# takah29/2d-fluid-simulator

Hardware: AMD Instinct MI355X
Metric: simulation steps/sec + Poisson-sweep HBM GB/s (% roofline), res 4096², 1/2/4/8 GPU (higher is better)
Workload: dtype f32; 1 GPU; bc=5 res=4096 (8192x4096 cells) scheme=cip vc=5.0 RB-SOR(1.3, 2 iters) Re=1e+06 dt=0.05/res; BASELINE.json configs[2]; cells=33554432, fluid_cells=22424499, parallelism=y-slab x1

## Files before the change

### 2d-fluid-simulator_amd/csrc/fs_core.hip

```cpp
#include <algorithm>
#include <cstdio>
#include <cstdlib>
#include <cstring>
#include <cxxabi.h>
#include <mutex>
#include <numeric>
#include <type_traits>
#include <unordered_map>

#include "fs_launch.h"
#include "fs_tracer.h"

namespace fs {

static thread_local std::string g_err;
void set_error(const std::string &msg) { g_err = msg; }
int no_variant(const char *name)
{
    set_error(std::string(name) + ": no kernel variant for these arguments");
    return FS_ERR_UNSUPPORTED;
}
int hip_fail(hipError_t e, const char *what, const char *file, int line)
{
    char buf[512];
// ... 88 lines not shown
        c->prof_ms[r.name_id] += ms;
        c->prof_pool.push_back(r.start);
        c->prof_pool.push_back(r.stop);
    }
    c->prof_recs.clear();
    return FS_OK;
}

const fs_ctx::TileList *tile_list(fs_ctx *c, TileSpec spec)
{
    if (c->act.quad.empty() || !tile_spec_ok(spec, c->rows)) return nullptr;
    const fs_ctx::TileKey key = spec.key();
    auto it = c->tile_lists.find(key);
    if (it != c->tile_lists.end()) return it->second.d ? &it->second : nullptr;
    if (c->capturing || c->tape_rec || c->tile_lists.size() >= 512) { ++c->tile_list_misses; return nullptr; }
    const TileWords h = build_tile_list(spec, c->act.of(spec.lanes).data(), c->X, c->rows);
    fs_ctx::TileList tl;
    if (h.needed) {
        if (hipMalloc(&tl.d, h.words.size() * sizeof(uint32_t)) == hipSuccess &&
            hipMemcpyAsync(tl.d, h.words.data(), h.words.size() * sizeof(uint32_t), hipMemcpyHostToDevice, c->stream) == hipSuccess &&
            hipStreamSynchronize(c->stream) == hipSuccess)
            { tl.per_xcd = h.per_xcd; tl.count = h.count; }
        else { if (tl.d) hipFree(tl.d); tl.d = nullptr; }
    }
    auto &slot = c->tile_lists[key] = tl;
    return slot.d ? &slot : nullptr;
}

static void tile_lists_free(fs_ctx *c)
{
    for (auto &kv : c->tile_lists) if (kv.second.d) hipFree(kv.second.d);
    c->tile_lists.clear();
}

int check_rows(const fs_ctx *c, int jb, int je)
{
    if (!(0 <= jb && jb <= je && je <= c->rows)) {
// ... 474 lines not shown
    FS_HIP(hipSetDevice(ctx->device));
    FS_HIP(hipMemsetAsync(ctx->d_mask, 1, (size_t)ctx->rows * ctx->Pm, ctx->stream));
    int rc = upload_global(ctx, ctx->d_mask, 1, 1, mask_xy, ctx->Pm);
    if (rc) return rc;
    rc = build_bc_ops(ctx, mask_xy);
    if (rc) return rc;
    if (!ctx->d_bcmap) FS_HIP(hipMalloc(&ctx->d_bcmap, (size_t)ctx->rows * ctx->Pm));
    if (!ctx->d_lazyflags) FS_HIP(hipMalloc(&ctx->d_lazyflags, (size_t)std::max(ctx->nwx, 1) * ctx->rows));
    FS_HIP(hipMemsetAsync(ctx->d_bcmap, 0, (size_t)ctx->rows * ctx->Pm, ctx->stream));
    FS_HIP(hipMemsetAsync(ctx->d_lazyflags, 63, (size_t)std::max(ctx->nwx, 1) * ctx->rows, ctx->stream));
    rc = upload_global(ctx, ctx->d_bcmap, 1, 1, ctx->h_bcmap.data(), ctx->Pm);
    for (auto &gexec : ctx->graphs) if (gexec) { hipGraphExecDestroy(gexec); gexec = nullptr; }
    for (auto &tp : ctx->tapes) if (tp) { delete tp; tp = nullptr; }
    tile_lists_free(ctx);
    ctx->act.clear();
    if (ctx->X % 2 == 0 && ctx->tile_list_mask && ctx->rows <= TILE_MAX_ROWS)
        ctx->act = activity_maps(mask_xy, ctx->h_bcmap.data(), ctx->X, ctx->Y, ctx->rows, ctx->y0 - ctx->halo);
    std::vector<uint8_t>().swap(ctx->h_bcmap);
    if (rc) return rc;
    if (ctx->X % 4 == 0) {
        klaunch(k_lazy_flags, dim3((ctx->nwx * ctx->rows + 3) / 4), dim3(256), ctx->stream, ctx->grid(), ctx->nwx, ctx->d_bcmap, ctx->d_lazyflags);
        FS_HIP(hipGetLastError());
        const size_t cap = (size_t)ctx->nwx * ctx->rows;
        if (!ctx->d_pairlist) FS_HIP(hipMalloc(&ctx->d_pairlist, (2 * cap + 2) * sizeof(uint32_t)));
        unsigned *d_count = (unsigned *)(ctx->d_pairlist + 2 * cap);
        FS_HIP(hipMemsetAsync(d_count, 0, 2 * sizeof(unsigned), ctx->stream));
        klaunch(k_pair_list, dim3((ctx->nwx * ctx->rows + 3) / 4), dim3(256), ctx->stream, ctx->grid(), ctx->nwx, (uint8_t *)ctx->d_lazyflags,
                           ctx->d_pairlist, ctx->d_pairlist + cap, d_count);
        FS_HIP(hipGetLastError());
        unsigned n[2] = {0, 0};
        FS_HIP(hipMemcpyAsync(n, d_count, 2 * sizeof(unsigned), hipMemcpyDeviceToHost, ctx->stream));
        FS_HIP(hipStreamSynchronize(ctx->stream));
// ... 1189 lines not shown
    FS_REQUIRE(ctx->span_ev[0], "fs_span_end without fs_span_begin");
    FS_HIP(hipEventRecord(ctx->span_ev[1], ctx->stream));
    FS_HIP(hipEventSynchronize(ctx->span_ev[1]));
    float f = 0.f;
    FS_HIP(hipEventElapsedTime(&f, ctx->span_ev[0], ctx->span_ev[1]));
    *ms = f;
    return FS_OK;
}

int fs_prof_reset(fs_ctx *ctx)
{
    FS_REQUIRE(ctx, "ctx is null");
    int rc = prof_drain(ctx); if (rc) return rc;
    std::fill(ctx->prof_launches.begin(), ctx->prof_launches.end(), 0);
    std::fill(ctx->prof_ms.begin(), ctx->prof_ms.end(), 0.0);
    return FS_OK;
}

int fs_prof_count(fs_ctx *ctx, int *n)
{
    FS_REQUIRE(ctx && n, "null argument");
    int rc = prof_drain(ctx); if (rc) return rc;
    *n = (int)ctx->prof_names.size();
    return FS_OK;
}

int fs_prof_get(fs_ctx *ctx, int idx, char *name, int name_cap, int *launches, double *total_ms)
{
    FS_REQUIRE(ctx, "ctx is null");
    FS_REQUIRE(idx >= 0 && idx < (int)ctx->prof_names.size(), "bad profile index");
// ... 38 lines not shown
```

### 2d-fluid-simulator_amd/csrc/fs_host.h

```cpp
#pragma once
#include <hip/hip_runtime.h>
#include <stdint.h>

#include <array>
#include <cmath>
#include <functional>
#include <map>
#include <set>
#include <string>
#include <vector>

#include "../../include/fs_hip.h"
#include "fs_device.h"
#include "fs_kernels.h"
#include "fs_march.h"
#include "fs_rbpair.h"
#include "fs_jquad.h"
#include "fs_k34n.h"
#include "fs_history.h"

namespace fs {

void set_error(const std::string &msg);
int hip_fail(hipError_t e, const char *what, const char *file, int line);
// ... 98 lines not shown
    std::set<fs_tracer *> tracers;
    std::vector<std::function<void()>> deferred_release;
    void release_deferred()
    {
        for (auto &release : deferred_release) release();
        deferred_release.clear();
    }
    bool use_march = true;
    bool use_pairs = true;
    int fuse_k2 = 2;
    bool limit_gate = true;
    int stack_mask = 0;

    int tile_list_mask = 1 | 2 | 4 | 8 | 32;
    fs::ActivityMaps act;
    struct TileList { uint32_t *d = nullptr; int per_xcd = 0; int count = 0; };
    using TileKey = decltype(fs::TileSpec().key());
    std::map<TileKey, TileList> tile_lists;

    fs::Grid grid() const
    {
        fs::Grid g;
        g.tiles = nullptr;
        g.X = X; g.P = P; g.Pm = Pm; g.rows = rows;
        int jlo = halo - y0, jhi = halo - y0 + (Y - 1);
        g.jlo = jlo < 0 ? 0 : jlo;
        g.jhi = jhi > rows - 1 ? rows - 1 : jhi;
        g.ybase = y0 - halo;
        g.mask = d_mask;
        return g;
    }
// ... 136 lines not shown
```

### 2d-fluid-simulator_amd/csrc/fs_k234.h

```cpp
#pragma once
#include <type_traits>

#include "fs_k34n.h"

namespace fs {

#if defined(__HIP_DEVICE_COMPILE__)
#define FS_PIN_LANE_OFFSET(i) asm volatile("" : "+v"(i))
#else
#define FS_PIN_LANE_OFFSET(i) (void)(i)
#endif

template <int RT> struct K234State {
    v2f Nn[RT + 4], Fc[RT + 4], GX[RT + 2], GY[RT + 2];
};

template <int c, int RT, int DM>
__device__ __forceinline__ void k234_nonadv(const Grid &g, const Konst<float> &k, const LaneMapN<2> &lm, int i0, int j0,
                                            const float *fc, const float *pc, K234State<RT> &st)
{
    using T = float;
    constexpr int N = 2;
    v2f F[RT + 6];
    v2f P[RT + 6];
// ... 129 lines not shown
    const int lane = threadIdx.x & 63;
    cip_k34_pk_core<2, c, RT, DM, false, false>(g, k, lm, i0, j0, je, MaskPacked{nwbits >> 2, flbits}, st.Nn, st.Fc, st.GX, st.GY, AdvLds<RT>{xch + (1 - c) * (RT + 2), lane}, out, gxo, gyo, hot, gxc, gyc);
}

#ifndef FS_K234_BND_WAVES
#define FS_K234_BND_WAVES 4
#endif
template <int RT, int DM>
__global__ __launch_bounds__(128, FS_K234_BND_WAVES) void k_cip_step_bnd(Grid g, Konst<float> k, int nbx, int nby, int jb, int je,
                                                      float *out, float *gxo, float *gyo, float *fn, const float *fc, const float *pc,
                                                      const float *gxc, const float *gyc, unsigned *hot, unsigned *hot_fn)
{
    constexpr int N = 2, HL = 2, OW = 64 - 2 * HL;
    __shared__ v2f xch[2 * (RT + 2)][64];
    int wx, ty, cg;
    if (!band_coords<1>(g, nbx, nby, wx, ty, cg)) return;
    if (!(wx * OW < g.X / N && jb + ty * RT < je)) return;
    const int c = __builtin_amdgcn_readfirstlane((int)(threadIdx.x >> 6));
    const LaneMapN<N> lm = lane_map_n<N, HL>(g, wx);
    const int i0 = lm.i0, j0 = jb + ty * RT;
    K234State<RT> st;
    unsigned nwbits, flbits;
    if (c == 0) k234_bnd_phase1<0, RT, DM>(g, k, lm, i0, j0, je, fn, fc, pc, gxc, gyc, hot_fn, st, nwbits, flbits, xch);
    else        k234_bnd_phase1<1, RT, DM>(g, k, lm, i0, j0, je, fn, fc, pc, gxc, gyc, hot_fn, st, nwbits, flbits, xch);
    __syncthreads();
    if (c == 0) k234_bnd_phase2<0, RT, DM>(g, k, lm, i0, j0, je, out, gxo, gyo, gxc, gyc, hot, st, nwbits, flbits, xch);
    else        k234_bnd_phase2<1, RT, DM>(g, k, lm, i0, j0, je, out, gxo, gyo, gxc, gyc, hot, st, nwbits, flbits, xch);
}

template <int RT, int DM>
__global__ __launch_bounds__(128, 4) void k_cip_step_all(Grid g, Konst<float> k, int nbx, int nby, int jb, int je,
                                                         float *out, float *gxo, float *gyo, float *fn, const float *fc, const float *pc,
                                                         const float *gxc, const float *gyc, unsigned *hot, unsigned *hot_fn)
{
    constexpr int N = 2, HL = 2, OW = 64 - 2 * HL;
    __shared__ v2f xch[2 * (RT + 2)][64];
    int wx, ty, cg;
    unsigned cls = 0u;
    if (!band_coords<1>(g, nbx, nby, wx, ty, cg, 0, &cls)) return;
    if (!(wx * OW < g.X / N && jb + ty * RT < je)) return;
    const int c = __builtin_amdgcn_readfirstlane((int)(threadIdx.x >> 6));
    const LaneMapN<N> lm_in = lane_map_n<N, HL>(g, wx);
    const int i0 = lm_in.i0, j0 = jb + ty * RT;
    K234State<RT> st;
    if (cls & 1u) {
        const LaneMapN<N> lm{lm_in.i0, lm_in.owner, false, false};
        if (c == 0) k234_phase1<0, RT, DM>(g, k, lm, i0, j0, fc, pc, gxc, gyc, st, xch);
        else        k234_phase1<1, RT, DM>(g, k, lm, i0, j0, fc, pc, gxc, gyc, st, xch);
        __syncthreads();
        if (c == 0) k234_phase2<0, RT, DM>(g, k, lm, i0, j0, je, out, gxo, gyo, hot, st, xch);
        else        k234_phase2<1, RT, DM>(g, k, lm, i0, j0, je, out, gxo, gyo, hot, st, xch);
    } else {
        unsigned nwbits, flbits;
        if (c == 0) k234_bnd_phase1<0, RT, DM>(g, k, lm_in, i0, j0, je, fn, fc, pc, gxc, gyc, hot_fn, st, nwbits, flbits, xch);
        else        k234_bnd_phase1<1, RT, DM>(g, k, lm_in, i0, j0, je, fn, fc, pc, gxc, gyc, hot_fn, st, nwbits, flbits, xch);
        __syncthreads();
        if (c == 0) k234_bnd_phase2<0, RT, DM>(g, k, lm_in, i0, j0, je, out, gxo, gyo, gxc, gyc, hot, st, nwbits, flbits, xch);
// ... 116 lines not shown
```

### 2d-fluid-simulator_amd/csrc/fs_launch.h

```cpp
#pragma once
#include <algorithm>
#include <cstdio>
#include <cstdlib>
#include <cstring>
#include <type_traits>

#include "fs_host.h"
#include "fs_pick.h"

namespace fs {

hipEvent_t prof_event(fs_ctx *c);


template <typename F>
inline bool launched(const F &f)
{
    if constexpr (std::is_void<decltype(f())>::value) { f(); return true; }
    else return f();
}
int no_variant(const char *name);

template <typename F>
inline int launch(fs_ctx *c, const char *name, F &&f)
// ... 78 lines not shown
    klaunch(kern, og.grid, dim3(og.threads), stream, og.g, k, og.nbx, og.nby, args...);
}
template <typename... P, typename... A>
inline void klaunch(void (*kern)(Grid, int, int, P...), const OvGrid &og, hipStream_t stream, A... args)
{
    klaunch(kern, og.grid, dim3(og.threads), stream, og.g, og.nbx, og.nby, args...);
}
enum { XCD_RBSOR = 1, XCD_VORT = 2, XCD_ADVECT = 4, XCD_NONADV = 8, XCD_GRAD = 16, XCD_JACOBI = 32 };

struct TileLaunch {
    int family, lanes;
    int rt = 1, zgroups = 1, wgw = 4;
    bool compact = true;
    int cls = TILES_ALL, reach = 0, parent_rt = 0;
    bool slab_classes = false;

    TileLaunch rows(int n) const { TileLaunch l = *this; l.rt = n; return l; }
    TileLaunch channel_groups(int n) const { TileLaunch l = *this; l.zgroups = n; return l; }
    TileLaunch waves(int n) const { TileLaunch l = *this; l.wgw = n; return l; }
    TileLaunch dense_if(bool dense) const { TileLaunch l = *this; l.compact = !dense; return l; }
    TileLaunch hints_within(int reach_) const { TileLaunch l = *this; l.cls = TILES_ALL; l.reach = reach_; return l; }
    TileLaunch plain_within(int reach_) const { TileLaunch l = *this; l.cls = TILES_PLAIN; l.reach = reach_; return l; }
    TileLaunch boundary_within(int reach_) const { TileLaunch l = *this; l.cls = TILES_BOUNDARY; l.reach = reach_; return l; }
    TileLaunch mixed_within(int reach_) const { TileLaunch l = *this; l.cls = TILES_MIXED; l.reach = reach_; return l; }
    TileLaunch parent_rows(int n) const { TileLaunch l = *this; l.parent_rt = n; return l; }
    TileLaunch classes_on_slabs(bool on) const { TileLaunch l = *this; l.slab_classes = on; return l; }
};
static inline TileLaunch tiles(int family, int lanes) { return TileLaunch{family, lanes}; }

static inline TileLaunch one_wave_where_hinted(const fs_ctx *c, TileLaunch l)
{
    if (c->dtype == 0 && (l.family & (XCD_RBSOR | XCD_JACOBI)) && l.wgw == 4 && l.cls == TILES_ALL && l.reach > 0 && l.compact) l.wgw = 1;
    return l;
}
static inline TileSpec list_spec(const fs_ctx *c, const TileLaunch &l, int jb, int je)
{
    TileSpec s;
    s.lanes = l.lanes; s.rt = l.rt; s.wgw = l.wgw; s.cls = l.cls; s.reach = l.reach; s.parent_rt = l.parent_rt; s.jb = jb; s.je = je;
    const int waves = geo_waves(c->X, l.lanes), tile_rows = (je - jb + l.rt - 1) / l.rt;
    s.stacked = (c->stack_mask & l.family) != 0 && l.wgw > 1;
    s.nbx = s.stacked ? waves : (waves + l.wgw - 1) / l.wgw;
    s.nby = s.stacked ? (tile_rows + l.wgw - 1) / l.wgw : tile_rows;
    constexpr int xg = 8;
    s.group = s.stacked ? std::max(1, xg / l.wgw) : xg;
    return s;
}
const fs_ctx::TileList *tile_list(fs_ctx *c, TileSpec spec);

static inline OvGrid ov_grid(fs_ctx *c, int jb, int je, const TileLaunch &asked)
{
    const TileLaunch l = one_wave_where_hinted(c, asked);
    const TileSpec s = list_spec(c, l, jb, je);
    OvGrid o;
// ... 38 lines not shown
```

### 2d-fluid-simulator_amd/csrc/fs_march.h

```cpp
#pragma once
#include "fs_device.h"
#include "fs_kernels.h"
#include "fs_tiles.h"

namespace fs {

template <typename T> struct Quad;
template <> struct Quad<float> { using type = float4; };
template <> struct Quad<double> { using type = double4; };

__device__ __forceinline__ float lane_prev(float x)
{ return __int_as_float(__builtin_amdgcn_update_dpp(0, __float_as_int(x), 0x138, 0xf, 0xf, true)); }
__device__ __forceinline__ float lane_next(float x)
{ return __int_as_float(__builtin_amdgcn_update_dpp(0, __float_as_int(x), 0x130, 0xf, 0xf, true)); }
__device__ __forceinline__ double lane_prev(double x)
{
    const int lo = __builtin_amdgcn_update_dpp(0, __double2loint(x), 0x138, 0xf, 0xf, true), hi = __builtin_amdgcn_update_dpp(0, __double2hiint(x), 0x138, 0xf, 0xf, true);
    return __hiloint2double(hi, lo);
}
__device__ __forceinline__ double lane_next(double x)
{
    const int lo = __builtin_amdgcn_update_dpp(0, __double2loint(x), 0x130, 0xf, 0xf, true), hi = __builtin_amdgcn_update_dpp(0, __double2hiint(x), 0x130, 0xf, 0xf, true);
    return __hiloint2double(hi, lo);
}
// ... 69 lines not shown
__device__ __forceinline__ void source_from(const Konst<T> &k, T vxE, T vxW, T vyE, T vyW, T vxN, T vxS, T vyN, T vyS, T &s2, T &s3)
{
    T sxx = vxE - vxW, sxy = vyE - vyW, syx = vxN - vxS, syy = vyN - vyS;
    s2 = ((sxx * sxx + syy * syy) + (syx * sxy)) / (T)8.0;
    s3 = cdiv<DM>(k.dx * (sxx + syy), k.eight_dt, k.r_eight_dt);
}

struct LaneMap {
    int i0;
    bool owner;
    bool at_lo;
    bool at_hi;
};
constexpr int FS_CG_INNER = 1 << 22;
template <int ZG = 1>
__device__ __forceinline__ bool band_coords(const Grid &g, int nbx, int nby_packed, int &bx, int &by, int &cg, int zoff = 0, unsigned *cls = nullptr)
{
    if (cls) *cls = 0u;
    if (g.tiles) {
        const int t = (int)blockIdx.x >> 3, xcd = (int)blockIdx.x & 7;
        const int k = ZG == 1 ? t : t / ZG;
        cg = ZG == 1 ? 0 : t - k * ZG;
        const uint32_t e = g.tiles[k * 8 + xcd];
        bx = tile_entry_bx(e);
        by = tile_entry_by(e);
        if (cls) *cls = tile_entry_hints(e);
        return e != TILE_PAD;
    }
    const int nby = nby_packed & 0x3fffff, FS_XCD_GROUP = (nby_packed >> 24) + 1;
    const int xcd = blockIdx.x & 7;
    int ly;
    if (ZG > 1 && (nby_packed & FS_CG_INNER)) {
        const int t = (int)blockIdx.x >> 3;
        bx = t / ZG;
        cg = t - bx * ZG;
        ly = (int)blockIdx.y;
    } else {
        bx = blockIdx.x >> 3;
        ly = ZG == 1 ? (int)blockIdx.y : (int)blockIdx.y / ZG;
        cg = ZG == 1 ? 0 : (int)blockIdx.y - ly * ZG;
    }
// ... 726 lines not shown
```

### 2d-fluid-simulator_amd/csrc/fs_pressure.hip

```cpp
#include "fs_launch.h"

using namespace fs;

template <bool SW, bool HV, typename T>
static bool launch_pair(fs_ctx *ctx, const OvGrid &og, int rt, int row_begin, int row_end, fs_field *pn, const fs_field *pc, const fs_field *src)
{
    const uint32_t *list = ctx->d_pairlist + (HV ? (size_t)ctx->nwx * ctx->rows : 0);
    const int nlist = ctx->n_pairlist[HV ? 1 : 0];
    const int per_slice = (int)(og.grid.x * og.grid.y), blocks = nlist, zoff = (blocks + per_slice - 1) / per_slice;
    const dim3 grid(og.grid.x, og.grid.y, og.grid.z + zoff);
    return pick<2, 3>(rt, [&](auto RT) {
        klaunch(k_jacobi_pair<RT, SW, HV, T>, grid, dim3(256), ctx->stream, og.g, og.nbx, og.nby, row_begin, row_end, (const uint8_t *)ctx->d_bcmap,
                (const uint8_t *)ctx->d_lazyflags, list, nlist, zoff, (T *)pn->d, (const T *)pc->d, (const T *)src->d);
    });
}

template <bool SRC, typename T>
static int launch_jacobi(fs_ctx *ctx, const char *name, const Konst<T> &k, int jb, int je, T *pn, const T *pc, const T *vs)
{
    if constexpr (!SRC && std::is_same<T, float>::value) {
        if (ctx->use_pairs) {
            const OvGrid og = ov_grid(ctx, jb, je, tiles(XCD_JACOBI, LANES_PAIR_WIDE).rows(4).hints_within(1));
            const int dm = dm_const(ctx, k);
            return launch(ctx, name, [=] { return with_dm_const<T>(dm, [&](auto DM) { klaunch(k_jacobi_ov2<4, DM>, og, ctx->stream, k, jb, je, pn, pc, vs); }); });
// ... 200 lines not shown
            const OvGrid ogb = ov_grid(ctx, row_begin, row_end, tiles(XCD_RBSOR, LANES_PAIR).rows(2).waves(1).boundary_within(4).parent_rows(4));
            if (ogp.g.tiles && ogb.g.tiles) {
                int rc = launch(ctx, "rbsor_pair", [=] { return run(ogp, Int<4>{}, Int<3>{}, Bool<false>{}); });
                if (rc) return rc;
                return launch(ctx, "rbsor_pair_bnd", [=] { return run(ogb, Int<2>{}, Int<2>{}, Bool<false>{}); });
            }
        }
        const OvGrid og = ov_grid(ctx, row_begin, row_end, tiles(XCD_RBSOR, LANES_PAIR).rows(2).dense_if(full).hints_within(4));
        return launch(ctx, "rbsor_pair", [=] { return pick_bool(full != 0, [&](auto FULL) { return run(og, Int<2>{}, Int<2>{}, FULL); }); });
    }
    using T = float;
    auto k = make_konst<T>(ctx, dt, dx, 1.0, 0.0, omega);
    const int dm = dm_const(ctx, k);
    const int rt = full || !small_tiles(ctx) ? 4 : 2;
    if (!full && split_launch(ctx, (size_t)ctx->X * ctx->Y, (size_t)1 << 20)) {
        const OvGrid og = ov_grid(ctx, row_begin, row_end, tiles(XCD_RBSOR, LANES_PAIR).rows(8).waves(1).mixed_within(4).parent_rows(16).classes_on_slabs(ctx->halo != 0));
        if (og.g.tiles) {
            return launch(ctx, "rbsor_pair", [=] {
                return pick<0, 1>(par0, [&](auto PAR) { return with_dm_const<T>(dm, [&](auto DM) {
                    klaunch(k_rbsor_pair_all<2, PAR, DM, T>, og.with_threads(128), ctx->stream, k, row_begin, row_end, (const uint8_t *)ctx->d_bcmap, (T *)pc_out->d, (T *)pn_out->d,
                            (const T *)pc->d, (const T *)pn->d, (const T *)vc->d);
                }); });
            });
        }
    }
    const OvGrid og = ov_grid(ctx, row_begin, row_end, tiles(XCD_RBSOR, LANES_PAIR).rows(rt).dense_if(full).hints_within(4));
    auto run = [=](auto RT, auto DM, auto FULL) {
        constexpr int tile = decltype(RT)::value, mode = decltype(DM)::value;
        constexpr bool carry = decltype(FULL)::value;
        return pick<0, 1>(par0, [&](auto PAR) {
            klaunch(k_rbsor_pair<2, tile, PAR, mode, 2, carry, T>, og, ctx->stream, k, row_begin, row_end, (const uint8_t *)ctx->d_bcmap, (T *)pc_out->d, (T *)pn_out->d,
// ... 76 lines not shown
```

### 2d-fluid-simulator_amd/csrc/fs_rbpair.h

```cpp
#pragma once
#include "fs_march.h"

namespace fs {

#ifndef FS_RBP_MIRROR
#define FS_RBP_MIRROR 1
#endif

template <typename T, int N> struct LV { T a[N]; };
template <typename T, int N> struct LVec;
template <> struct LVec<float, 4> { using type = float4; };
template <> struct LVec<float, 2> { using type = float2; };
template <> struct LVec<double, 2> { using type = double2; };
template <int N> struct LMaskWord;
template <> struct LMaskWord<4> { using type = uint32_t; };
template <> struct LMaskWord<2> { using type = uint16_t; };

template <typename T, int N>
__device__ __forceinline__ LV<T, N> lv_load(const T *row, int i0)
{
    const typename LVec<T, N>::type q = load_row_quad<typename LVec<T, N>::type, T>(row, i0);
    LV<T, N> r;
    if constexpr (N == 4) { r.a[0] = q.x; r.a[1] = q.y; r.a[2] = q.z; r.a[3] = q.w; }
    else { r.a[0] = q.x; r.a[1] = q.y; }
// ... 105 lines not shown
template <int N> struct LaneMapN { int i0; bool owner, at_lo, at_hi; };
template <int N, int HL = 4 / N>
__device__ __forceinline__ LaneMapN<N> lane_map_n(const Grid &g, int wave)
{
    constexpr int OW = 64 - 2 * HL;
    const int lane = threadIdx.x & 63, nu = g.X / N;
    int q = wave * OW - HL + lane;
    LaneMapN<N> m;
    m.owner = lane >= HL && lane < 64 - HL && q >= 0 && q < nu;
    q = q < 0 ? 0 : (q > nu - 1 ? nu - 1 : q);
    m.i0 = q * N;
    m.at_lo = q == 0;
    m.at_hi = q == nu - 1;
    return m;
}
template <typename T, int N> __device__ __forceinline__ T lv_left(const LaneMapN<N> &m, const LV<T, N> &v)
{ const T l = lane_prev(v.a[N - 1]); return m.at_lo ? v.a[0] : l; }
template <typename T, int N> __device__ __forceinline__ T lv_right(const LaneMapN<N> &m, const LV<T, N> &v)
{ const T r = lane_next(v.a[0]); return m.at_hi ? v.a[N - 1] : r; }

template <int N>
__device__ __forceinline__ bool tile_coords_n(const Grid &g, int nbx, int nby_packed, int jb, int je, int rt, int &wave_x, int &tile_y, bool *plain_hint = nullptr, bool *bnd_fluid = nullptr)
{
    constexpr int OW = 64 - 2 * (4 / N);
    int bx, by, cg;
    unsigned cls = 0u;
    if (!band_coords<1>(g, nbx, nby_packed, bx, by, cg, 0, plain_hint ? &cls : nullptr)) return false;
    const int w = __builtin_amdgcn_readfirstlane((int)(threadIdx.x >> 6)), nw = blockDim.x >> 6;
    if (plain_hint) *plain_hint = ((cls >> w) & 1u) != 0u;
    if (bnd_fluid) *bnd_fluid = nw == 1 && (cls & 2u) != 0u;
// ... 210 lines not shown
        if ((PARW + w) & 1) rbp_relax<1, 0>(k, lm, ALL, P3[w - UP], P3[w], P3[w + UP], S2[w], S3[w], P4[w]);
        else                rbp_relax<0, 0>(k, lm, ALL, P3[w - UP], P3[w], P3[w + UP], S2[w], S3[w], P4[w]);
    }
    if (lm.owner) {
#pragma unroll
        for (int w = 4; w <= W - 2; ++w) {
            lv_store_row<1, T, N>(C, g, 0, i0, FS_ROW(w), P4[w]);
            lv_store_row<1, T, N>(D, g, 0, i0, FS_ROW(w), P2[w]);
        }
    }
#undef FS_ROW
}

template <int N, int RT, int PAR0, int DM, int PATH, bool FULL, typename T>
__device__ __forceinline__ void rbsor_pair_wave_at(const Grid &g, const Konst<T> &k, int wx, int ty, bool hint, bool bnd_fluid, int jb, int je,
                                                   const uint8_t *bcmap, T *C, T *D, const T *A, const T *B, const T *v)
{
    constexpr int W = RT + 8;
    const LaneMapN<N> lm = lane_map_n<N>(g, wx);
    const int i0 = lm.i0, j0 = jb + ty * RT;
    unsigned fl[W];
    bool plain = PATH == 3 || hint;
    if (!plain && bnd_fluid) {
#pragma unroll
        for (int w = 0; w < W; ++w) fl[w] = lv_sel_fluid<N>(lv_bytes<N>(g.mask, g, i0, clampy(g, j0 - 4 + w)));
    } else if (!plain) {
        bool own_fluid = false, all_fluid = true;
#pragma unroll
        for (int w = 0; w < W; ++w) {
            fl[w] = lv_sel_fluid<N>(lv_bytes<N>(g.mask, g, i0, clampy(g, j0 - 4 + w)));
            all_fluid = all_fluid && fl[w] == (1u << N) - 1u;
            if (w >= 4 && w <= W - 5 && j0 - 4 + w < je) own_fluid = own_fluid || (lm.owner && fl[w] != 0u);
        }
        if (!FULL && !__any(own_fluid)) {
// ... 20 lines not shown
                                                const uint8_t *bcmap, T *C, T *D, const T *A, const T *B, const T *v)
{
    int wx, ty;
    bool hint = false, bnd_fluid = false;
    if (!tile_coords_n<N>(g, nbx, nby, jb, je, RT, wx, ty, PATH == 2 && !FULL ? &hint : nullptr, PATH == 2 && !FULL ? &bnd_fluid : nullptr)) return;
    rbsor_pair_wave_at<N, RT, PAR0, DM, PATH, FULL, T>(g, k, wx, ty, hint, bnd_fluid, jb, je, bcmap, C, D, A, B, v);
}

template <int N, int PAR0, int DM, typename T>
__global__ __launch_bounds__(128) void k_rbsor_pair_all(Grid g, Konst<T> k, int nbx, int nby, int jb, int je, const uint8_t *bcmap, T *C, T *D, const T *A, const T *B, const T *v)
{
    constexpr int RT = 8;
    __shared__ typename LVec<T, N>::type xch[3][2][64];
    constexpr int OW = 64 - 2 * (4 / N);
    int wx, ty, cg;
    unsigned cls = 0u;
    if (!band_coords<1>(g, nbx, nby, wx, ty, cg, 0, &cls)) return;
    if (!(wx * OW < g.X / N && jb + ty * RT < je)) return;
    const int w = __builtin_amdgcn_readfirstlane((int)(threadIdx.x >> 6));
    if (cls & 1u) {
        const LaneMapN<N> lm = lane_map_n<N>(g, wx);
        const int j0 = jb + ty * RT;
        if (w == 0) rbsor_pair_stack_tile<N, RT, PAR0, DM, false, T>(g, k, lm, lm.i0, j0, C, D, A, B, v, xch, 0);
        else        rbsor_pair_stack_tile<N, RT, PAR0, DM, true, T>(g, k, lm, lm.i0, j0 + RT, C, D, A, B, v, xch, 1);
    } else {
        const int t4 = ty * 2 + w;
        if (jb + t4 * 4 >= je) return;
        rbsor_pair_wave_at<N, 4, PAR0, DM, 2, false, T>(g, k, wx, t4, false, ((cls >> (1 + w)) & 1u) != 0u, jb, je, bcmap, C, D, A, B, v);
    }
}

template <int N, int RT, int PAR0, int DM, int PATH, bool FULL, typename T>
__global__ __launch_bounds__(256, (PATH == 3 && sizeof(T) == 4 ? 4 : 1)) void k_rbsor_pair(Grid g, Konst<T> k, int nbx, int nby, int jb, int je,
                                                    const uint8_t *bcmap, T *C, T *D, const T *A, const T *B, const T *v)
{
    static_assert(RT % 2 == 0, "the row parity of a tile is a launch constant only for even tile heights");
    rbsor_pair_wave<N, RT, PAR0, DM, PATH, FULL, T>(g, k, nbx, nby, jb, je, bcmap, C, D, A, B, v);
}


}
```

### 2d-fluid-simulator_amd/csrc/fs_tiles.h

```cpp
#pragma once
#include <stdint.h>

#include <algorithm>
#include <array>
#include <cstddef>
#include <vector>

namespace fs {

constexpr uint32_t TILE_PAD = 0xffffffffu;
constexpr int TILE_MAX_NBX = 0xfff, TILE_MAX_NBY = 0xffff, TILE_MAX_ROWS = 0xffff;
constexpr uint32_t tile_entry(uint32_t hints, int by, int bx) { return (hints << 28) | ((uint32_t)by << 12) | (uint32_t)bx; }
constexpr int tile_entry_bx(uint32_t e) { return (int)(e & 0xfffu); }
constexpr int tile_entry_by(uint32_t e) { return (int)((e >> 12) & 0xffffu); }
constexpr unsigned tile_entry_hints(uint32_t e) { return e >> 28; }
constexpr uint32_t HINT_PLAIN = 1u, HINT_FLUID = 2u;

enum { LANES_PAIR = 2, LANES_PAIR_WIDE = 3, LANES_QUAD = 4 };
constexpr int geo_cells(int lanes) { return lanes == LANES_QUAD ? 4 : 2; }
constexpr int geo_owners(int lanes) { return lanes == LANES_PAIR ? 60 : 62; }
constexpr int geo_width(int lanes) { return geo_cells(lanes) * geo_owners(lanes); }
constexpr int geo_halo(int lanes) { return (64 - geo_owners(lanes)) / 2 * geo_cells(lanes); }
inline int geo_waves(int X, int lanes) { return (X / geo_cells(lanes) + geo_owners(lanes) - 1) / geo_owners(lanes); }

// ... 31 lines not shown
    return m;
}

enum { TILES_ALL = 0, TILES_PLAIN = 1, TILES_BOUNDARY = 2, TILES_MIXED = 3 };
struct TileSpec {
    int lanes = LANES_QUAD;
    int rt = 1;
    int wgw = 4;
    bool stacked = false;
    int group = 8;
    int cls = TILES_ALL;
    int reach = 0;
    int parent_rt = 0;
    int jb = 0, je = 0;
    int nbx = 0, nby = 0;

    std::array<int, 10> key() const { return {{lanes, rt, stacked ? 1 : 0, group, cls, reach, wgw, parent_rt, jb, je}}; }
};
inline bool tile_spec_ok(TileSpec &s, int rows)
{
    if (s.parent_rt == s.rt) s.parent_rt = 0;
    if (s.nbx > TILE_MAX_NBX || s.nby > TILE_MAX_NBY || rows > TILE_MAX_ROWS || s.lanes > LANES_QUAD) return false;
    if (s.parent_rt && (s.wgw != 1 || s.parent_rt % s.rt != 0 || s.parent_rt > 64)) return false;
    if (s.cls == TILES_MIXED && !(s.rt == 8 && s.parent_rt == 16 && s.wgw == 1 && s.lanes == LANES_PAIR)) return false;
    return true;
}

struct TileWords {
    std::vector<uint32_t> words;
    int per_xcd = 0, count = 0;
    bool needed = false;
};

namespace tiles_detail {

struct Act {
    const uint8_t *a; int waves, rows;
    bool any(int wx0, int wx1, int j0, int j1, uint8_t bit) const
    {
        for (int wx = wx0; wx < wx1; ++wx)
            for (int j = j0; j < j1; ++j)
                if (a[(size_t)wx * rows + j] & bit) return true;
        return false;
    }
};
struct Tile { int bx, by, wx0, wx1, j0, j1; };

// ... 70 lines not shown
            const size_t n = std::min(per[d].size() - target, target - per[r].size());
            per[r].insert(per[r].end(), per[d].end() - n, per[d].end());
            per[d].resize(per[d].size() - n);
        }
}
inline std::vector<uint32_t> interleave(const PerXcd &per, size_t K)
{
    std::vector<uint32_t> h(K * 8, TILE_PAD);
    for (int xcd = 0; xcd < 8; ++xcd)
        for (size_t k = 0; k < per[xcd].size(); ++k) h[k * 8 + xcd] = per[xcd][k];
    return h;
}

}

inline TileWords build_tile_list(const TileSpec &s, const uint8_t *act_map, int X, int rows)
{
    using namespace tiles_detail;
    const Act act{act_map, geo_waves(X, s.lanes), rows};
    const auto entry = s.cls == TILES_MIXED ? entry_mixed : (s.cls == TILES_ALL ? entry_all : entry_split);
    PerXcd per;
    const int groups = (s.nby + s.group - 1) / s.group;
    for (int xcd = 0; xcd < 8; ++xcd)
        for (int g = xcd; g < groups; g += 8)
            for (int bx = 0; bx < s.nbx; ++bx)
                for (int by = g * s.group; by < std::min(s.nby, (g + 1) * s.group); ++by) {
                    uint32_t e;
                    if (entry(s, act, workgroup(s, act, bx, by), e)) per[xcd].push_back(e);
                }
    size_t K = 0, total = 0;
    bool any_hint = s.cls == TILES_MIXED;
    for (auto &v : per) {
        total += v.size();
        if (s.cls == TILES_ALL) for (uint32_t e : v) any_hint = any_hint || tile_entry_hints(e) != 0u;
    }
    if ((s.cls == TILES_ALL || s.cls == TILES_MIXED) && any_hint && s.wgw == 1) masked_first(per);
    balance_xcds(per, total);
    for (auto &v : per) K = std::max(K, v.size());
    TileWords out;
    out.needed = K > 0 && (s.cls != TILES_ALL || any_hint || total < (size_t)s.nbx * s.nby);
    if (out.needed) { out.words = interleave(per, K); out.per_xcd = (int)K; out.count = (int)total; }
    return out;
}

}
```

### 2d-fluid-simulator_amd/csrc/fs_tiles_host.cpp

```cpp
#include <cstring>

#include "fs_pick.h"
#include "fs_tiles.h"

extern "C" {

void fs_tiles_activity(const uint8_t *mask_xy, const uint8_t *bcmap_xy, int X, int Y, int rows, int g0, uint8_t *quad, uint8_t *pair, uint8_t *pair_wide)
{
    const fs::ActivityMaps m = fs::activity_maps(mask_xy, bcmap_xy, X, Y, rows, g0);
    std::memcpy(quad, m.quad.data(), m.quad.size());
    std::memcpy(pair, m.pair.data(), m.pair.size());
    std::memcpy(pair_wide, m.pair_wide.data(), m.pair_wide.size());
}

int fs_tiles_build(const int *spec, const uint8_t *act, int X, int rows, uint32_t *words, int capacity, int *per_xcd, int *count)
{
    fs::TileSpec s;
    s.lanes = spec[0]; s.rt = spec[1]; s.wgw = spec[2]; s.stacked = spec[3] != 0; s.group = spec[4]; s.cls = spec[5]; s.reach = spec[6];
    s.parent_rt = spec[7]; s.jb = spec[8]; s.je = spec[9]; s.nbx = spec[10]; s.nby = spec[11];
    *per_xcd = *count = 0;
    if (!fs::tile_spec_ok(s, rows)) return -1;
    const fs::TileWords t = fs::build_tile_list(s, act, X, rows);
    if ((int)t.words.size() > capacity) return -2;
    if (!t.words.empty()) std::memcpy(words, t.words.data(), t.words.size() * sizeof(uint32_t));
    *per_xcd = t.per_xcd; *count = t.count;
    return (int)t.words.size();
}

int fs_pick_dm(int family, int f32, int dm)
{
    int got = -1;
    auto note = [&](auto DM) { got = DM; };
    bool found = false;
    if (f32) found = family == 0 ? fs::with_dm_const<float>(dm, note) : (family == 1 ? fs::with_dm_dx<float>(dm, note) : fs::with_dm_all<float>(dm, note));
    else found = family == 0 ? fs::with_dm_const<double>(dm, note) : (family == 1 ? fs::with_dm_dx<double>(dm, note) : fs::with_dm_all<double>(dm, note));
    return found ? got : -1;
}
int fs_pick_dm_table(int family, int f32, int dm)
{
    return family == 0 ? fs::dm_pick_const(f32 != 0, dm) : (family == 1 ? fs::dm_pick_dx(f32 != 0, dm) : fs::dm_pick_all(f32 != 0, dm));
}
int fs_pick_probe(int flag, int v, int *called)
{
// ... 6 lines not shown
```

### 2d-fluid-simulator_amd/csrc/fs_transport.hip

```cpp
#include "fs_launch.h"
#include "fs_k234.h"

using namespace fs;

template <int C, bool CLAMP>
static int launch_k34(fs_ctx *ctx, const char *name, const char *name_bnd, double dt, double dx, fs_field *f_out, fs_field *gx_out, fs_field *gy_out,
                      const fs_field *fn, const fs_field *fc, const fs_field *gxc, const fs_field *gyc, const fs_field *v, int full, int jb, int je)
{
    using T = float;
    auto k = make_konst<T>(ctx, dt, dx, 1.0);
    const int dm = dm_dx(ctx, k);
    const size_t cells = (size_t)ctx->X * ctx->rows;
    const int N = ctx->X % 4 != 0 || C == 3 ? 2 : (cells >= ((size_t)1 << 23) || cells < ((size_t)1 << 21) ? 2 : 4);
    const int RT = N == 4 ? 2 : (cells >= ((size_t)1 << 23) ? 4 : (small_tiles(ctx) && !full && C == 3 ? 1 : 2)), geo = N == 2 ? LANES_PAIR_WIDE : LANES_QUAD;
    auto run = [=](const OvGrid &og, auto NN, auto R, auto PL) {
        constexpr int nn = decltype(NN)::value, r = decltype(R)::value;
        constexpr bool plain = decltype(PL)::value;
        return with_dm_dx<T>(dm, [&](auto DM) {
            klaunch(k_cip_grad_advect_n<C, nn, r, DM, plain, CLAMP, T>, og, ctx->stream, k, jb, je, (T *)f_out->d, (T *)gx_out->d, (T *)gy_out->d, (const T *)fn->d,
                    (const T *)fc->d, (const T *)gxc->d, (const T *)gyc->d, v ? (const T *)v->d : (const T *)nullptr, f_out->hot, (const uint8_t *)ctx->d_bcmap, full);
        });
    };
    auto any = [=](const OvGrid &og, auto PL) {
        return N == 4 ? run(og, Int<4>{}, Int<2>{}, PL) : (RT == 4 ? run(og, Int<2>{}, Int<4>{}, PL) : run(og, Int<2>{}, Int<2>{}, PL));
// ... 249 lines not shown
int fs_cip_step(fs_ctx *ctx, double dt, double dx, double re, fs_field *v_out, fs_field *gx_out, fs_field *gy_out, fs_field *fn,
                const fs_field *fc, const fs_field *pc, const fs_field *gxc, const fs_field *gyc, int full, int row_begin, int row_end)
{
    FS_REQUIRE(ctx, "ctx is null");
    FS_FIELD(v_out, 2); FS_FIELD(gx_out, 2); FS_FIELD(gy_out, 2); FS_FIELD(fn, 2); FS_FIELD(fc, 2); FS_FIELD(pc, 1); FS_FIELD(gxc, 2); FS_FIELD(gyc, 2);
    FS_REQUIRE(v_out != fn && v_out != fc && gx_out != gxc && gy_out != gyc && fn != fc, "outputs must not alias inputs");
    FS_REQUIRE(ctx->use_pairs, "the fused gradient+advection pass needs an even X (use the two-kernel form)");
    FS_ROWS();
    if (ctx->dtype != 0) { set_error("the fused gradient+advection pass exists for f32 (f64: the two-kernel form)"); return FS_ERR_UNSUPPORTED; }
    using T = float;
    constexpr int RT = 4;
    const bool slab = ctx->halo != 0;
    if (cip_step_multi_part(ctx) && !full && cip_step_rows(ctx, row_begin, row_end)) {
        auto k = make_konst<T>(ctx, dt, dx, re);
        const int dm = dm_all(ctx, k);
        const TileLaunch step_tiles = tiles(XCD_ADVECT, LANES_PAIR).waves(1);
        auto tiles_of = [=](const OvGrid &og, auto kern) {
            klaunch(kern, og.with_threads(128), ctx->stream, k, row_begin, row_end, (T *)v_out->d, (T *)gx_out->d, (T *)gy_out->d, (T *)fn->d, (const T *)fc->d, (const T *)pc->d,
                    (const T *)gxc->d, (const T *)gyc->d, v_out->hot, fn->hot);
        };
        if (ctx->fuse_k2 >= 2) {
            if (small_tiles(ctx)) {
                const OvGrid oga = ov_grid(ctx, row_begin, row_end, step_tiles.rows(2).hints_within(2));
                if (oga.g.tiles) return launch(ctx, "cip_step", [=] { return with_dm_all<T>(dm, [&](auto DM) { tiles_of(oga, k_cip_step_all<2, DM>); }); });
            }
            const OvGrid oga = ov_grid(ctx, row_begin, row_end, step_tiles.rows(RT).hints_within(2));
            if (oga.g.tiles) return launch(ctx, "cip_step", [=] { return with_dm_all<T>(dm, [&](auto DM) { tiles_of(oga, k_cip_step_all<RT, DM>); }); });
        }
        const OvGrid ogp = ov_grid(ctx, row_begin, row_end, step_tiles.rows(RT).plain_within(2).classes_on_slabs(slab));
        const OvGrid ogb = ov_grid(ctx, row_begin, row_end, step_tiles.rows(RT).boundary_within(2).classes_on_slabs(slab));
        if (ogp.g.tiles && ogb.g.tiles) {
// ... 126 lines not shown
```

Measured before the change: 1931 steps/s.

## Add per-tile live-lane ranges to skip wall-only lanes in boundary tiles

The host tile-list builder now computes, for each non-plain tile, the contiguous range of wave lanes whose column neighbourhood (within a reach) contains any non-wall cell. It stores these lo/hi words after the tile list on the device. The RB-SOR pair kernel and the CIP step kernels read the word through band_coords and use a new lane map that clamps addresses and clears ownership outside the live range. This is meant to cut loads and stores in solid-obstacle regions of boundary tiles. The cost is a host-side copy of the mask, extra list-building work, and one more global load per tile; correctness depends on the reach values chosen.

Result: faster. 1956 steps/s, median of 6 (+1.3%).

```diff
diff --git a/2d-fluid-simulator_amd/csrc/fs_core.hip b/2d-fluid-simulator_amd/csrc/fs_core.hip
--- a/2d-fluid-simulator_amd/csrc/fs_core.hip
+++ b/2d-fluid-simulator_amd/csrc/fs_core.hip
@@ -126,13 +126,17 @@
     auto it = c->tile_lists.find(key);
     if (it != c->tile_lists.end()) return it->second.d ? &it->second : nullptr;
     if (c->capturing || c->tape_rec || c->tile_lists.size() >= 512) { ++c->tile_list_misses; return nullptr; }
-    const TileWords h = build_tile_list(spec, c->act.of(spec.lanes).data(), c->X, c->rows);
+    LiveMask lm;
+    lm.mask_xy = c->h_mask.empty() ? nullptr : c->h_mask.data(); lm.Y = c->Y; lm.g0 = c->y0 - c->halo;
+    const TileWords h = build_tile_list(spec, c->act.of(spec.lanes).data(), c->X, c->rows, lm);
     fs_ctx::TileList tl;
     if (h.needed) {
-        if (hipMalloc(&tl.d, h.words.size() * sizeof(uint32_t)) == hipSuccess &&
-            hipMemcpyAsync(tl.d, h.words.data(), h.words.size() * sizeof(uint32_t), hipMemcpyHostToDevice, c->stream) == hipSuccess &&
+        const size_t bytes = h.words.size() * sizeof(uint32_t);
+        if (hipMalloc(&tl.d, 2 * bytes) == hipSuccess &&
+            hipMemcpyAsync(tl.d, h.words.data(), bytes, hipMemcpyHostToDevice, c->stream) == hipSuccess &&
+            hipMemcpyAsync(tl.d + h.words.size(), h.live.data(), bytes, hipMemcpyHostToDevice, c->stream) == hipSuccess &&
             hipStreamSynchronize(c->stream) == hipSuccess)
-            { tl.per_xcd = h.per_xcd; tl.count = h.count; }
+            { tl.per_xcd = h.per_xcd; tl.count = h.count; tl.masked_lanes = h.masked_lanes; tl.dead_lanes = h.dead_lanes; }
         else { if (tl.d) hipFree(tl.d); tl.d = nullptr; }
     }
     auto &slot = c->tile_lists[key] = tl;
@@ -637,8 +641,11 @@
     for (auto &tp : ctx->tapes) if (tp) { delete tp; tp = nullptr; }
     tile_lists_free(ctx);
     ctx->act.clear();
-    if (ctx->X % 2 == 0 && ctx->tile_list_mask && ctx->rows <= TILE_MAX_ROWS)
+    std::vector<uint8_t>().swap(ctx->h_mask);
+    if (ctx->X % 2 == 0 && ctx->tile_list_mask && ctx->rows <= TILE_MAX_ROWS) {
         ctx->act = activity_maps(mask_xy, ctx->h_bcmap.data(), ctx->X, ctx->Y, ctx->rows, ctx->y0 - ctx->halo);
+        ctx->h_mask.assign(mask_xy, mask_xy + (size_t)ctx->X * ctx->Y);
+    }
     std::vector<uint8_t>().swap(ctx->h_bcmap);
     if (rc) return rc;
     if (ctx->X % 4 == 0) {
@@ -1858,6 +1865,7 @@
     int rc = prof_drain(ctx); if (rc) return rc;
     std::fill(ctx->prof_launches.begin(), ctx->prof_launches.end(), 0);
     std::fill(ctx->prof_ms.begin(), ctx->prof_ms.end(), 0.0);
+    for (auto &ks : ctx->prof_kernels) ks.clear();
     return FS_OK;
 }
 
diff --git a/2d-fluid-simulator_amd/csrc/fs_host.h b/2d-fluid-simulator_amd/csrc/fs_host.h
--- a/2d-fluid-simulator_amd/csrc/fs_host.h
+++ b/2d-fluid-simulator_amd/csrc/fs_host.h
@@ -136,7 +136,8 @@
 
     int tile_list_mask = 1 | 2 | 4 | 8 | 32;
     fs::ActivityMaps act;
-    struct TileList { uint32_t *d = nullptr; int per_xcd = 0; int count = 0; };
+    std::vector<uint8_t> h_mask;
+    struct TileList { uint32_t *d = nullptr; int per_xcd = 0; int count = 0; long long masked_lanes = 0, dead_lanes = 0; };
     using TileKey = decltype(fs::TileSpec().key());
     std::map<TileKey, TileList> tile_lists;
 
diff --git a/2d-fluid-simulator_amd/csrc/fs_k234.h b/2d-fluid-simulator_amd/csrc/fs_k234.h
--- a/2d-fluid-simulator_amd/csrc/fs_k234.h
+++ b/2d-fluid-simulator_amd/csrc/fs_k234.h
@@ -167,10 +167,11 @@
     constexpr int N = 2, HL = 2, OW = 64 - 2 * HL;
     __shared__ v2f xch[2 * (RT + 2)][64];
     int wx, ty, cg;
-    if (!band_coords<1>(g, nbx, nby, wx, ty, cg)) return;
+    unsigned live = LIVE_ALL;
+    if (!band_coords<1>(g, nbx, nby, wx, ty, cg, 0, nullptr, &live)) return;
     if (!(wx * OW < g.X / N && jb + ty * RT < je)) return;
     const int c = __builtin_amdgcn_readfirstlane((int)(threadIdx.x >> 6));
-    const LaneMapN<N> lm = lane_map_n<N, HL>(g, wx);
+    const LaneMapN<N> lm = lane_map_live<N, HL>(g, wx, live);
     const int i0 = lm.i0, j0 = jb + ty * RT;
     K234State<RT> st;
     unsigned nwbits, flbits;
@@ -189,11 +190,11 @@
     constexpr int N = 2, HL = 2, OW = 64 - 2 * HL;
     __shared__ v2f xch[2 * (RT + 2)][64];
     int wx, ty, cg;
-    unsigned cls = 0u;
-    if (!band_coords<1>(g, nbx, nby, wx, ty, cg, 0, &cls)) return;
+    unsigned cls = 0u, live = LIVE_ALL;
+    if (!band_coords<1>(g, nbx, nby, wx, ty, cg, 0, &cls, &live)) return;
     if (!(wx * OW < g.X / N && jb + ty * RT < je)) return;
     const int c = __builtin_amdgcn_readfirstlane((int)(threadIdx.x >> 6));
-    const LaneMapN<N> lm_in = lane_map_n<N, HL>(g, wx);
+    const LaneMapN<N> lm_in = lane_map_live<N, HL>(g, wx, live);
     const int i0 = lm_in.i0, j0 = jb + ty * RT;
     K234State<RT> st;
     if (cls & 1u) {
diff --git a/2d-fluid-simulator_amd/csrc/fs_launch.h b/2d-fluid-simulator_amd/csrc/fs_launch.h
--- a/2d-fluid-simulator_amd/csrc/fs_launch.h
+++ b/2d-fluid-simulator_amd/csrc/fs_launch.h
@@ -116,6 +116,7 @@
     bool compact = true;
     int cls = TILES_ALL, reach = 0, parent_rt = 0;
     bool slab_classes = false;
+    int live = 0;
 
     TileLaunch rows(int n) const { TileLaunch l = *this; l.rt = n; return l; }
     TileLaunch channel_groups(int n) const { TileLaunch l = *this; l.zgroups = n; return l; }
@@ -126,6 +127,7 @@
     TileLaunch boundary_within(int reach_) const { TileLaunch l = *this; l.cls = TILES_BOUNDARY; l.reach = reach_; return l; }
     TileLaunch mixed_within(int reach_) const { TileLaunch l = *this; l.cls = TILES_MIXED; l.reach = reach_; return l; }
     TileLaunch parent_rows(int n) const { TileLaunch l = *this; l.parent_rt = n; return l; }
+    TileLaunch live_within(int reach_) const { TileLaunch l = *this; l.live = reach_; return l; }
     TileLaunch classes_on_slabs(bool on) const { TileLaunch l = *this; l.slab_classes = on; return l; }
 };
 static inline TileLaunch tiles(int family, int lanes) { return TileLaunch{family, lanes}; }
@@ -138,7 +140,7 @@
 static inline TileSpec list_spec(const fs_ctx *c, const TileLaunch &l, int jb, int je)
 {
     TileSpec s;
-    s.lanes = l.lanes; s.rt = l.rt; s.wgw = l.wgw; s.cls = l.cls; s.reach = l.reach; s.parent_rt = l.parent_rt; s.jb = jb; s.je = je;
+    s.lanes = l.lanes; s.rt = l.rt; s.wgw = l.wgw; s.cls = l.cls; s.reach = l.reach; s.parent_rt = l.parent_rt; s.jb = jb; s.je = je; s.live = l.live;
     const int waves = geo_waves(c->X, l.lanes), tile_rows = (je - jb + l.rt - 1) / l.rt;
     s.stacked = (c->stack_mask & l.family) != 0 && l.wgw > 1;
     s.nbx = s.stacked ? waves : (waves + l.wgw - 1) / l.wgw;
diff --git a/2d-fluid-simulator_amd/csrc/fs_march.h b/2d-fluid-simulator_amd/csrc/fs_march.h
--- a/2d-fluid-simulator_amd/csrc/fs_march.h
+++ b/2d-fluid-simulator_amd/csrc/fs_march.h
@@ -107,7 +107,7 @@
 };
 constexpr int FS_CG_INNER = 1 << 22;
 template <int ZG = 1>
-__device__ __forceinline__ bool band_coords(const Grid &g, int nbx, int nby_packed, int &bx, int &by, int &cg, int zoff = 0, unsigned *cls = nullptr)
+__device__ __forceinline__ bool band_coords(const Grid &g, int nbx, int nby_packed, int &bx, int &by, int &cg, int zoff = 0, unsigned *cls = nullptr, unsigned *live = nullptr)
 {
     if (cls) *cls = 0u;
     if (g.tiles) {
@@ -118,6 +118,7 @@
         bx = tile_entry_bx(e);
         by = tile_entry_by(e);
         if (cls) *cls = tile_entry_hints(e);
+        if (live) *live = g.tiles[(int)gridDim.x / ZG + k * 8 + xcd];
         return e != TILE_PAD;
     }
     const int nby = nby_packed & 0x3fffff, FS_XCD_GROUP = (nby_packed >> 24) + 1;
diff --git a/2d-fluid-simulator_amd/csrc/fs_pressure.hip b/2d-fluid-simulator_amd/csrc/fs_pressure.hip
--- a/2d-fluid-simulator_amd/csrc/fs_pressure.hip
+++ b/2d-fluid-simulator_amd/csrc/fs_pressure.hip
@@ -238,7 +238,7 @@
     const int dm = dm_const(ctx, k);
     const int rt = full || !small_tiles(ctx) ? 4 : 2;
     if (!full && split_launch(ctx, (size_t)ctx->X * ctx->Y, (size_t)1 << 20)) {
-        const OvGrid og = ov_grid(ctx, row_begin, row_end, tiles(XCD_RBSOR, LANES_PAIR).rows(8).waves(1).mixed_within(4).parent_rows(16).classes_on_slabs(ctx->halo != 0));
+        const OvGrid og = ov_grid(ctx, row_begin, row_end, tiles(XCD_RBSOR, LANES_PAIR).rows(8).waves(1).mixed_within(4).parent_rows(16).live_within(4).classes_on_slabs(ctx->halo != 0));
         if (og.g.tiles) {
             return launch(ctx, "rbsor_pair", [=] {
                 return pick<0, 1>(par0, [&](auto PAR) { return with_dm_const<T>(dm, [&](auto DM) {
diff --git a/2d-fluid-simulator_amd/csrc/fs_rbpair.h b/2d-fluid-simulator_amd/csrc/fs_rbpair.h
--- a/2d-fluid-simulator_amd/csrc/fs_rbpair.h
+++ b/2d-fluid-simulator_amd/csrc/fs_rbpair.h
@@ -143,6 +143,23 @@
     m.at_hi = q == nu - 1;
     return m;
 }
+template <int N, int HL = 4 / N>
+__device__ __forceinline__ LaneMapN<N> lane_map_live(const Grid &g, int wave, unsigned live)
+{
+    constexpr int OW = 64 - 2 * HL;
+    const int lane = threadIdx.x & 63, nu = g.X / N;
+    const int lo = (int)(live & 0xffu), hi = (int)((live >> 8) & 0xffu);
+    const int q = wave * OW - HL + lane;
+    const int from = lane < lo ? lo : (lane > hi - 1 ? hi - 1 : lane);
+    int ql = wave * OW - HL + from;
+    ql = ql < 0 ? 0 : (ql > nu - 1 ? nu - 1 : ql);
+    LaneMapN<N> m;
+    m.owner = lane >= HL && lane < 64 - HL && q >= 0 && q < nu && lane >= lo && lane < hi;
+    m.i0 = ql * N;
+    m.at_lo = q <= 0;
+    m.at_hi = q >= nu - 1;
+    return m;
+}
 template <typename T, int N> __device__ __forceinline__ T lv_left(const LaneMapN<N> &m, const LV<T, N> &v)
 { const T l = lane_prev(v.a[N - 1]); return m.at_lo ? v.a[0] : l; }
 template <typename T, int N> __device__ __forceinline__ T lv_right(const LaneMapN<N> &m, const LV<T, N> &v)
@@ -383,10 +400,10 @@
 
 template <int N, int RT, int PAR0, int DM, int PATH, bool FULL, typename T>
 __device__ __forceinline__ void rbsor_pair_wave_at(const Grid &g, const Konst<T> &k, int wx, int ty, bool hint, bool bnd_fluid, int jb, int je,
-                                                   const uint8_t *bcmap, T *C, T *D, const T *A, const T *B, const T *v)
+                                                   const uint8_t *bcmap, T *C, T *D, const T *A, const T *B, const T *v, unsigned live = LIVE_ALL)
 {
     constexpr int W = RT + 8;
-    const LaneMapN<N> lm = lane_map_n<N>(g, wx);
+    const LaneMapN<N> lm = lane_map_live<N>(g, wx, live);
     const int i0 = lm.i0, j0 = jb + ty * RT;
     unsigned fl[W];
     bool plain = PATH == 3 || hint;
@@ -437,8 +454,8 @@
     __shared__ typename LVec<T, N>::type xch[3][2][64];
     constexpr int OW = 64 - 2 * (4 / N);
     int wx, ty, cg;
-    unsigned cls = 0u;
-    if (!band_coords<1>(g, nbx, nby, wx, ty, cg, 0, &cls)) return;
+    unsigned cls = 0u, live = LIVE_ALL;
+    if (!band_coords<1>(g, nbx, nby, wx, ty, cg, 0, &cls, &live)) return;
     if (!(wx * OW < g.X / N && jb + ty * RT < je)) return;
     const int w = __builtin_amdgcn_readfirstlane((int)(threadIdx.x >> 6));
     if (cls & 1u) {
@@ -449,7 +466,7 @@
     } else {
         const int t4 = ty * 2 + w;
         if (jb + t4 * 4 >= je) return;
-        rbsor_pair_wave_at<N, 4, PAR0, DM, 2, false, T>(g, k, wx, t4, false, ((cls >> (1 + w)) & 1u) != 0u, jb, je, bcmap, C, D, A, B, v);
+        rbsor_pair_wave_at<N, 4, PAR0, DM, 2, false, T>(g, k, wx, t4, false, ((cls >> (1 + w)) & 1u) != 0u, jb, je, bcmap, C, D, A, B, v, live);
     }
 }
 
diff --git a/2d-fluid-simulator_amd/csrc/fs_tiles.h b/2d-fluid-simulator_amd/csrc/fs_tiles.h
--- a/2d-fluid-simulator_amd/csrc/fs_tiles.h
+++ b/2d-fluid-simulator_amd/csrc/fs_tiles.h
@@ -69,8 +69,9 @@
     int parent_rt = 0;
     int jb = 0, je = 0;
     int nbx = 0, nby = 0;
-
-    std::array<int, 10> key() const { return {{lanes, rt, stacked ? 1 : 0, group, cls, reach, wgw, parent_rt, jb, je}}; }
+    int live = 0;
+
+    std::array<int, 11> key() const { return {{lanes, rt, stacked ? 1 : 0, group, cls, reach, wgw, parent_rt, jb, je, live}}; }
 };
 inline bool tile_spec_ok(TileSpec &s, int rows)
 {
@@ -83,9 +84,40 @@
 
 struct TileWords {
     std::vector<uint32_t> words;
+    std::vector<uint32_t> live;
     int per_xcd = 0, count = 0;
+    long long masked_lanes = 0, dead_lanes = 0;
     bool needed = false;
 };
+
+constexpr uint32_t LIVE_ALL = 64u << 8;
+constexpr uint32_t live_word(int lo, int hi) { return (uint32_t)lo | ((uint32_t)hi << 8); }
+constexpr int live_lo(uint32_t w) { return (int)(w & 0xffu); }
+constexpr int live_hi(uint32_t w) { return (int)((w >> 8) & 0xffu); }
+struct LiveMask { const uint8_t *mask_xy = nullptr; int Y = 0, g0 = 0; };
+
+inline void live_hull(const LiveMask &m, int X, int lanes, int reach, int wx, int j0, int j1, int &lo, int &hi)
+{
+    const int N = geo_cells(lanes), OW = geo_owners(lanes), HL = (64 - OW) / 2, nu = X / N;
+    const int ja = std::max(0, m.g0 + j0 - reach), jb = std::min(m.Y - 1, m.g0 + j1 - 1 + reach);
+    const int qa = std::min(std::max(wx * OW - HL, 0), nu - 1), qb = std::min(std::max(wx * OW - HL + 63, 0), nu - 1);
+    const int xa = std::max(0, qa * N - reach), xb = std::min(X - 1, qb * N + N - 1 + reach);
+    std::vector<int> open((size_t)(xb - xa + 2), 0);
+    for (int x = xa; x <= xb; ++x) {
+        const uint8_t *col = m.mask_xy + (size_t)x * m.Y;
+        bool wall = true;
+        for (int j = ja; j <= jb && wall; ++j) wall = col[j] == 1;
+        open[x - xa + 1] = open[x - xa] + (wall ? 0 : 1);
+    }
+    lo = 64; hi = 0;
+    for (int l = 0; l < 64; ++l) {
+        const int q = std::min(std::max(wx * OW - HL + l, 0), nu - 1);
+        const int x0 = std::max(0, q * N - reach), x1 = std::min(X - 1, q * N + N - 1 + reach);
+        if (open[x1 - xa + 1] - open[x0 - xa] == 0) continue;
+        lo = std::min(lo, l); hi = l + 1;
+    }
+    if (hi == 0) lo = 0;
+}
 
 namespace tiles_detail {
 
@@ -186,7 +218,7 @@
 
 }
 
-inline TileWords build_tile_list(const TileSpec &s, const uint8_t *act_map, int X, int rows)
+inline TileWords build_tile_list(const TileSpec &s, const uint8_t *act_map, int X, int rows, const LiveMask &mask = LiveMask())
 {
     using namespace tiles_detail;
     const Act act{act_map, geo_waves(X, s.lanes), rows};
@@ -212,6 +244,19 @@
     TileWords out;
     out.needed = K > 0 && (s.cls != TILES_ALL || any_hint || total < (size_t)s.nbx * s.nby);
     if (out.needed) { out.words = interleave(per, K); out.per_xcd = (int)K; out.count = (int)total; }
+    out.live.assign(out.words.size(), LIVE_ALL);
+    if (s.live > 0 && mask.mask_xy && s.wgw == 1 && s.cls != TILES_PLAIN)
+        for (size_t q = 0; q < out.words.size(); ++q) {
+            const uint32_t e = out.words[q];
+            if (e == TILE_PAD || ((s.cls == TILES_ALL || s.cls == TILES_MIXED) && (tile_entry_hints(e) & HINT_PLAIN))) continue;
+            const Tile t = workgroup(s, act, tile_entry_bx(e), tile_entry_by(e));
+            int lo, hi;
+            live_hull(mask, X, s.lanes, s.live, t.wx0, t.j0, t.j1, lo, hi);
+            out.masked_lanes += 64;
+            if (hi == 0) continue;
+            out.live[q] = live_word(lo, hi);
+            out.dead_lanes += 64 - (hi - lo);
+        }
     return out;
 }
 
diff --git a/2d-fluid-simulator_amd/csrc/fs_tiles_host.cpp b/2d-fluid-simulator_amd/csrc/fs_tiles_host.cpp
--- a/2d-fluid-simulator_amd/csrc/fs_tiles_host.cpp
+++ b/2d-fluid-simulator_amd/csrc/fs_tiles_host.cpp
@@ -27,6 +27,29 @@
     return (int)t.words.size();
 }
 
+int fs_tiles_build_live(const int *spec, const uint8_t *act, int X, int rows, const uint8_t *mask_xy, int Y, int g0, int live_reach,
+                        uint32_t *words, uint32_t *live, int capacity, int *per_xcd, int *count, long long *lanes)
+{
+    fs::TileSpec s;
+    s.lanes = spec[0]; s.rt = spec[1]; s.wgw = spec[2]; s.stacked = spec[3] != 0; s.group = spec[4]; s.cls = spec[5]; s.reach = spec[6];
+    s.parent_rt = spec[7]; s.jb = spec[8]; s.je = spec[9]; s.nbx = spec[10]; s.nby = spec[11];
+    s.live = live_reach;
+    *per_xcd = *count = 0;
+    lanes[0] = lanes[1] = 0;
+    if (!fs::tile_spec_ok(s, rows)) return -1;
+    fs::LiveMask m;
+    m.mask_xy = mask_xy; m.Y = Y; m.g0 = g0;
+    const fs::TileWords t = fs::build_tile_list(s, act, X, rows, m);
+    if ((int)t.words.size() > capacity) return -2;
+    if (!t.words.empty()) {
+        std::memcpy(words, t.words.data(), t.words.size() * sizeof(uint32_t));
+        std::memcpy(live, t.live.data(), t.live.size() * sizeof(uint32_t));
+    }
+    *per_xcd = t.per_xcd; *count = t.count;
+    lanes[0] = t.masked_lanes; lanes[1] = t.dead_lanes;
+    return (int)t.words.size();
+}
+
 int fs_pick_dm(int family, int f32, int dm)
 {
     int got = -1;
diff --git a/2d-fluid-simulator_amd/csrc/fs_transport.hip b/2d-fluid-simulator_amd/csrc/fs_transport.hip
--- a/2d-fluid-simulator_amd/csrc/fs_transport.hip
+++ b/2d-fluid-simulator_amd/csrc/fs_transport.hip
@@ -287,7 +287,7 @@
     if (cip_step_multi_part(ctx) && !full && cip_step_rows(ctx, row_begin, row_end)) {
         auto k = make_konst<T>(ctx, dt, dx, re);
         const int dm = dm_all(ctx, k);
-        const TileLaunch step_tiles = tiles(XCD_ADVECT, LANES_PAIR).waves(1);
+        const TileLaunch step_tiles = tiles(XCD_ADVECT, LANES_PAIR).waves(1).live_within(3);
         auto tiles_of = [=](const OvGrid &og, auto kern) {
             klaunch(kern, og.with_threads(128), ctx->stream, k, row_begin, row_end, (T *)v_out->d, (T *)gx_out->d, (T *)gy_out->d, (T *)fn->d, (const T *)fc->d, (const T *)pc->d,
                     (const T *)gxc->d, (const T *)gyc->d, v_out->hot, fn->hot);
```
